# Vill-Lab/2023-TIFS-ISTVT

Hardware: AMD Instinct MI355X
Metric: clips/sec (BxTx3x224x224 fwd+bwd) (higher is better)
Workload: dtype bf16; 1 GPU; C2: B=32/GPU T=8 224x224 full ISTVT (Xception stem + 12-layer DSTTr) train step (fwd+bwd+grad all-reduce+SGD), random-init weights; global_batch=32, frames=8, size=224, depth=12, parallelism=dp1, early_allreduce=False, attn_fp8=False, dead_row_elimination=False, final_norm_class_rows_only=False, optimizer=SGD(momentum 0.9) fused, step_graphs=False

## Files before the change

2023-tifs-istvt_amd/build.py:

```python
import os
import subprocess
import sys
from concurrent.futures import ThreadPoolExecutor

HERE = os.path.dirname(os.path.abspath(__file__))
CSRC = os.path.join(HERE, 'csrc')
OBJ = os.path.join(CSRC, 'build')
LIB = os.path.join(HERE, 'libistvt_hip.so')
INCLUDE = os.path.join(os.path.dirname(HERE), 'include')
HIPCC = os.environ.get('HIPCC', '/opt/rocm/bin/hipcc')
FLAGS = ['--offload-arch=gfx950', '-O3', '-fPIC', '-std=c++17', '-Wno-unused-result', '-Wno-inline-asm', '-ffp-contract=fast', '-I', INCLUDE] + os.environ.get('ISTVT_EXTRA_HIPCC_FLAGS', '').split()


def _sources():
    return sorted(f for f in os.listdir(CSRC) if f.endswith('.hip'))


def _newest_header():
    headers = [os.path.join(CSRC, f) for f in os.listdir(CSRC) if f.endswith('.h')] + [os.path.join(INCLUDE, 'istvt_hip.h')]
    return max(os.path.getmtime(h) for h in headers)


def _compile(src):
    obj = os.path.join(OBJ, src[:-4] + '.o')
    path = os.path.join(CSRC, src)
    cmd = [HIPCC] + FLAGS + ['-Rpass-analysis=kernel-resource-usage', '-c', path, '-o', obj]
    r = subprocess.run(cmd, capture_output=True, text=True)
    if r.returncode != 0:
        raise RuntimeError('hipcc failed for %s:\n%s' % (src, r.stderr[-6000:]))
    _check_no_spills(src, r.stderr)
    return obj


NO_SPILL_KERNELS = ('gemm256q_kernel', 'gemm256t_kernel', 'gemm256t_group_kernel', 'pw_bwd_kernel')


def _check_no_spills(src, remarks):
    name = None
    for line in remarks.splitlines():
        if 'Function Name:' in line:
            name = line.split('Function Name:')[1].split()[0]
        elif 'ScratchSize [bytes/lane]:' in line and name and any(k in name for k in NO_SPILL_KERNELS):
            n = int(line.split('ScratchSize [bytes/lane]:')[1].split()[0])
            if n != 0:
                raise RuntimeError('%s: kernel %s spills %d bytes/lane to scratch; it must not (see build.py)' % (src, name, n))


def build(force: bool = False, verbose: bool = False) -> str:
    os.makedirs(OBJ, exist_ok=True)
    srcs = _sources()
    hdr = _newest_header()
    todo = []
    for s in srcs:
        obj = os.path.join(OBJ, s[:-4] + '.o')
        if force or not os.path.exists(obj) or os.path.getmtime(obj) < max(os.path.getmtime(os.path.join(CSRC, s)), hdr):
            todo.append(s)
    if verbose:
        print('compiling', todo)
    if todo:
        with ThreadPoolExecutor(max_workers=min(6, len(todo))) as ex:
            list(ex.map(_compile, todo))
    objs = [os.path.join(OBJ, s[:-4] + '.o') for s in srcs]
    if todo or not os.path.exists(LIB):
        cmd = [HIPCC, '--offload-arch=gfx950', '-shared', '-fPIC', '-o', LIB] + objs
        r = subprocess.run(cmd, capture_output=True, text=True)
        if r.returncode != 0:
            raise RuntimeError('link failed:\n' + r.stderr[-6000:])
    return LIB


if __name__ == '__main__':
    print(build(force='--force' in sys.argv, verbose=True))
```

2023-tifs-istvt_amd/csrc/conv_dense.hip:

```cpp
#include "common.h"
#include "u8_view.h"
#include <type_traits>

namespace {

__device__ __forceinline__ bf16x8 ld_frag(const bf16_t* p) { return *reinterpret_cast<const bf16x8*>(p); }
__device__ __forceinline__ bf16x8 zero_frag() {
    bf16x8 f;
#pragma unroll
    for (int i = 0; i < 8; ++i) f[i] = (bf16_t)0.0f;
    return f;
}
__device__ __forceinline__ f32x4 mma16(const bf16x8& a, const bf16x8& b, const f32x4& c) {
    return __builtin_amdgcn_mfma_f32_16x16x32_bf16(a, b, c, 0, 0, 0);
}

template <typename T>
__device__ __forceinline__ void conv1_mac_store(const float* v, const float* __restrict__ w, T* __restrict__ out) {
#pragma unroll
    for (int c8 = 0; c8 < 4; ++c8) {
        float o[8];
#pragma unroll
        for (int j = 0; j < 8; ++j) {
            const float* wc = w + (c8 * 8 + j) * 27;
            float a = 0.f;
#pragma unroll
            for (int k = 0; k < 27; ++k) a = fmaf(wc[k], v[k], a);
            o[j] = a;
        }
        store8(out + c8 * 8, o);
    }
}

template <typename T>
__global__ __launch_bounds__(256) void conv1_fwd_kernel(const float* __restrict__ x, const float* __restrict__ w,
                                                        T* __restrict__ u1, long Mo, int S, int Ho, int Wo) {
    const long m = (long)blockIdx.x * 256 + threadIdx.x;
    if (m >= Mo) return;
    const int xo = (int)(m % Wo), yo = (int)((m / Wo) % Ho);
    const long f = m / ((long)Wo * Ho);
    float v[27];
#pragma unroll
    for (int ci = 0; ci < 3; ++ci)
#pragma unroll
        for (int dy = 0; dy < 3; ++dy) {
            const float* row = x + ((f * 3 + ci) * S + 2 * yo + dy) * S + 2 * xo;
#pragma unroll
            for (int dx = 0; dx < 3; ++dx) v[ci * 9 + dy * 3 + dx] = row[dx];
        }
    conv1_mac_store(v, w, u1 + m * 32);
}

struct Conv1Mac {
    static __device__ __forceinline__ int slot(int dy, int dx, int ci) { return ci * 9 + dy * 3 + dx; }
    template <typename T>
    static __device__ __forceinline__ void emit(const float* v, const float* __restrict__ w, T* __restrict__ out) {
        int w0 = 0;
        asm volatile("" : "+s"(w0));
        conv1_mac_store(v, w + w0, out);
    }
};

struct Conv1Col {
    static __device__ __forceinline__ int slot(int dy, int dx, int ci) { return (dy * 3 + dx) * 3 + ci; }
    template <typename T>
    static __device__ __forceinline__ void emit(const float* v, const float*, T* __restrict__ out) {
#pragma unroll
        for (int c = 0; c < 4; ++c) {
            float t[8];
#pragma unroll
            for (int i = 0; i < 8; ++i) t[i] = c * 8 + i < 27 ? v[c * 8 + i] : 0.f;
            store8(out + c * 8, t);
        }
    }
};

template <typename Sink, typename T>
__global__ __launch_bounds__(256) void conv1_u8_kernel(const uint8_t* __restrict__ x, const int* __restrict__ view,
                                                       const float* __restrict__ mean, const float* __restrict__ stdv,
                                                       const float* __restrict__ w, T* __restrict__ out, long total,
                                                       int Hs, int Ws, int S, int Ho, int R, int ngroups) {
    extern __shared__ __align__(16) unsigned char smem[];
    float* lut = reinterpret_cast<float*>(smem);
    unsigned char* sb = smem + 3 * 256 * sizeof(float);
    const int tid = threadIdx.x;
    const int grp = (int)(blockIdx.x % ngroups);
    const long f = blockIdx.x / ngroups;
    const int yb = grp * R;
    const int rows = min(R, Ho - yb);
    const U8View vw = u8_view_of(view, f, Hs, Ws, S);
    u8_fill_lut(lut, mean, stdv, tid, 256);
    const int pitch = u8_row_pitch(S), rstride = Ws * 3;
    const long g0 = ((f * Hs + vw.y0 + 2 * yb) * (long)Ws + vw.x0) * 3;
    const int lead0 = u8_stage_rows(x, total, g0, rstride, 2 * rows + 1, S, sb, pitch, tid, 256);
    __syncthreads();
    const int nout = rows * Ho;
    for (int o = tid; o < nout; o += 256) {
        const int yl = o / Ho, xo = o - yl * Ho;
        float v[27];
#pragma unroll
        for (int dy = 0; dy < 3; ++dy) {
            const int rr = 2 * yl + dy;
            const unsigned char* row = sb + rr * pitch + u8_row_lead(lead0, rr, rstride);
#pragma unroll
            for (int dx = 0; dx < 3; ++dx) {
                const unsigned char* px = row + u8_view_px(2 * xo + dx, S, vw.flip);
#pragma unroll
                for (int ci = 0; ci < 3; ++ci) v[Sink::slot(dy, dx, ci)] = lut[ci * 256 + px[ci]];
            }
        }
        Sink::emit(v, w, out + ((f * Ho + yb) * (long)Ho + o) * 32);
    }
}

__global__ __launch_bounds__(256, 2) void conv2_fwd_kernel(const bf16_t* __restrict__ u1, const float* __restrict__ bnp,
                                                           const bf16_t* __restrict__ w, bf16_t* __restrict__ u2, long Mo,
                                                           int H, int W, int Ho, int Wo, int ngroups) {
    const int tid = threadIdx.x, lane = tid & 63, wave = tid >> 6;
    const int r = lane & 15, g = lane >> 4;
    __shared__ bf16x8 wl3[9 * 64];
    bf16x8 wf[9][3];
#pragma unroll
    for (int tap = 0; tap < 9; ++tap) {
#pragma unroll
        for (int nt = 0; nt < 3; ++nt)
            wf[tap][nt] = ld_frag(w + (16 * (r >> 2) + 4 * nt + (r & 3)) * 288 + tap * 32 + 8 * g);
        if (wave == 0) wl3[tap * 64 + lane] = ld_frag(w + (16 * (r >> 2) + 4 * 3 + (r & 3)) * 288 + tap * 32 + 8 * g);
    }
    __syncthreads();
    float mu[8], sc[8], be[8];
    load8(bnp + 8 * g, mu);
    load8(bnp + 2 * 32 + 8 * g, sc);
    load8(bnp + 3 * 32 + 8 * g, be);
    constexpr int RSEG = 9;
    const int nstrips = (Wo + 15) / 16, nsegs = (Ho + RSEG - 1) / RSEG;
    const long nitems = (long)(Mo / ((long)Ho * Wo)) * nstrips * nsegs;
    bf16x8 ring[3][3];
    for (long it = (long)blockIdx.x * 4 + wave; it < nitems; it += (long)gridDim.x * 4) {
        const int seg = (int)(it % nsegs);
        const int strip = (int)((it / nsegs) % nstrips);
        const long f = it / ((long)nsegs * nstrips);
        const int xo = strip * 16 + r;
        const bool ok = xo < Wo;
        const int xc = ok ? xo : Wo - 1;
        const int y0 = seg * RSEG;
        auto load_row = [&](int yi, bf16x8 (&dst)[3]) {
            const int yc = yi < H ? yi : H - 1;
            const bf16_t* sp = u1 + ((f * H + yc) * W + xc) * 32 + 8 * g;
#pragma unroll
            for (int dx = 0; dx < 3; ++dx) {
                const bf16x8 raw = ld_frag(sp + dx * 32);
#pragma unroll
                for (int j = 0; j < 8; ++j)
                    dst[dx][j] = (bf16_t)fmaxf(((float)raw[j] - mu[j]) * sc[j] + be[j], 0.f);
            }
        };
        load_row(y0, ring[0]);
        load_row(y0 + 1, ring[1]);
#pragma unroll
        for (int k = 0; k < RSEG; ++k) {
            const int yo = y0 + k;
            if (yo < Ho) {
                load_row(yo + 2, ring[(k + 2) % 3]);
                f32x4 acc[4];
#pragma unroll
                for (int nt = 0; nt < 4; ++nt) acc[nt] = f32x4{0.f, 0.f, 0.f, 0.f};
                int lo = lane;
                asm volatile("" : "+v"(lo));
#pragma unroll
                for (int dy = 0; dy < 3; ++dy)
#pragma unroll
                    for (int dx = 0; dx < 3; ++dx) {
                        const bf16x8& xf = ring[(k + dy) % 3][dx];
#pragma unroll
                        for (int nt = 0; nt < 3; ++nt) acc[nt] = mma16(wf[dy * 3 + dx][nt], xf, acc[nt]);
                        acc[3] = mma16(wl3[(dy * 3 + dx) * 64 + lo], xf, acc[3]);
                    }
                if (ok) {
                    bf16x8 o0, o1;
#pragma unroll
                    for (int i = 0; i < 4; ++i) {
                        o0[i] = (bf16_t)acc[0][i]; o0[4 + i] = (bf16_t)acc[1][i];
                        o1[i] = (bf16_t)acc[2][i]; o1[4 + i] = (bf16_t)acc[3][i];
                    }
                    bf16_t* dst = u2 + (((f * Ho + yo) * Wo) + xo) * 64 + 16 * g;
                    *reinterpret_cast<bf16x8*>(dst) = o0;
                    *reinterpret_cast<bf16x8*>(dst + 8) = o1;
                }
            }
        }
    }
}

__global__ __launch_bounds__(256, 2) void conv2_dgrad_kernel(const bf16_t* __restrict__ du2, const bf16_t* __restrict__ w,
                                                             const bf16_t* __restrict__ u1, const float* __restrict__ bnp,
                                                             bf16_t* __restrict__ dz1, long Mi, int H, int W, int Ho,
                                                             int Wo, int ngroups) {
    __shared__ bf16_t wt[9 * 32 * 64];
    const int tid = threadIdx.x, lane = tid & 63, wave = tid >> 6;
    const int r = lane & 15, g = lane >> 4;
    for (int i = tid; i < 64 * 36; i += 256) {
        const int co = i / 36, k8 = (i % 36) * 8;
        const bf16x8 v = ld_frag(w + co * 288 + k8);
#pragma unroll
        for (int j = 0; j < 8; ++j) wt[(k8 + j) * 64 + co] = v[j];
    }
    __syncthreads();
    bf16x8 wf[9][2][2];
#pragma unroll
    for (int tap = 3; tap < 9; ++tap)
#pragma unroll
        for (int ks = 0; ks < 2; ++ks)
#pragma unroll
            for (int nt = 0; nt < 2; ++nt)
                wf[tap][ks][nt] = ld_frag(wt + (tap * 32 + 8 * (r >> 2) + 4 * nt + (r & 3)) * 64 + 32 * ks + 8 * g);
    const int wrow = 8 * (r >> 2) + (r & 3), wcol = 8 * g;
    constexpr int RSEG = 9;
    const int nstrips = (W + 15) / 16, nsegs = (H + RSEG - 1) / RSEG;
    const long nitems = (long)(Mi / ((long)H * W)) * nstrips * nsegs;
    bf16x8 ring[3][3][2];
    for (long it = (long)blockIdx.x * 4 + wave; it < nitems; it += (long)gridDim.x * 4) {
        const int seg = (int)(it % nsegs);
        const int strip = (int)((it / nsegs) % nstrips);
        const long f = it / ((long)nsegs * nstrips);
        const int xi = strip * 16 + r;
        const int y0 = seg * RSEG;
        auto load_row = [&](int yo, bf16x8 (&dst)[3][2]) {
            const bool rowok = yo >= 0 && yo < Ho;
#pragma unroll
            for (int dx = 0; dx < 3; ++dx) {
                const int xo = xi - dx;
                const bool in = rowok && xo >= 0 && xo < Wo;
                const bf16_t* sp = du2 + ((f * Ho + yo) * Wo + xo) * 64 + 8 * g;
                dst[dx][0] = in ? ld_frag(sp) : zero_frag();
                dst[dx][1] = in ? ld_frag(sp + 32) : zero_frag();
            }
        };
        load_row(y0 - 2, ring[(RSEG * 3 - 2) % 3]);
        load_row(y0 - 1, ring[(RSEG * 3 - 1) % 3]);
#pragma unroll
        for (int k = 0; k < RSEG; ++k) {
            const int yi = y0 + k;
            if (yi < H) {
            load_row(yi, ring[k % 3]);
            const bool ok = xi < W;
            const long m = (f * H + yi) * W + (ok ? xi : W - 1);
            const bf16x8 uraw = ld_frag(u1 + m * 32 + 8 * g);
            f32x4 acc[2] = {f32x4{0.f, 0.f, 0.f, 0.f}, f32x4{0.f, 0.f, 0.f, 0.f}};
#pragma unroll
            for (int dyo = 2; dyo >= 1; --dyo) {
#pragma unroll
                for (int dx = 0; dx < 3; ++dx)
#pragma unroll
                    for (int ks = 0; ks < 2; ++ks)
#pragma unroll
                        for (int nt = 0; nt < 2; ++nt)
                            acc[nt] = mma16(wf[dyo * 3 + dx][ks][nt], ring[(k + 3 - dyo) % 3][dx][ks], acc[nt]);
            }
            int wo = wrow;
            asm volatile("" : "+v"(wo));
#pragma unroll
            for (int dx = 0; dx < 3; ++dx)
#pragma unroll
                for (int ks = 0; ks < 2; ++ks)
#pragma unroll
                    for (int nt = 0; nt < 2; ++nt)
                        acc[nt] = mma16(ld_frag(wt + (dx * 32 + wo + 4 * nt) * 64 + 32 * ks + wcol), ring[k % 3][dx][ks], acc[nt]);
            if (ok) {
                float mu[8], sc[8], be[8];
                load8(bnp + 8 * g, mu);
                load8(bnp + 2 * 32 + 8 * g, sc);
                load8(bnp + 3 * 32 + 8 * g, be);
                bf16x8 o;
#pragma unroll
                for (int j = 0; j < 8; ++j) {
                    const float z = ((float)uraw[j] - mu[j]) * sc[j] + be[j];
                    o[j] = (bf16_t)(z > 0.f ? acc[j >> 2][j & 3] : 0.f);
                }
                *reinterpret_cast<bf16x8*>(dz1 + m * 32 + 8 * g) = o;
            }
            }
        }
    }
}

constexpr int WG_PX = 32;
constexpr int DIMG_PITCH = 64 * 2 + 16;
constexpr int AIMG_PITCH = 32 * 2 + 16;
constexpr int AIMG_ROWS = WG_PX + 2;

__device__ __forceinline__ bf16x8 tr_frag(const char* img, int pitch, int k0, int col16, int r) {
    typedef short4v __attribute__((address_space(3))) * lds_ptr;
    typedef short short8v __attribute__((ext_vector_type(8)));
    const int q = r >> 2, pp = r & 3;
    const char* pa = img + (k0 + q) * pitch + (col16 + 4 * pp) * 2;
    const char* pb = pa + 4 * pitch;
    const short4v lo = __builtin_amdgcn_ds_read_tr16_b64_v4i16((lds_ptr)(pa));
    const short4v hi = __builtin_amdgcn_ds_read_tr16_b64_v4i16((lds_ptr)(pb));
    short8v s;
    s[0] = lo[0]; s[1] = lo[1]; s[2] = lo[2]; s[3] = lo[3]; s[4] = hi[0]; s[5] = hi[1]; s[6] = hi[2]; s[7] = hi[3];
    return __builtin_bit_cast(bf16x8, s);
}

__global__ __launch_bounds__(256) void conv2_wgrad_kernel(const bf16_t* __restrict__ du2, const bf16_t* __restrict__ u1,
                                                          const float* __restrict__ bnp, float* __restrict__ slabs,
                                                          int Fr, int H, int W, int Ho, int Wo, int nchunks) {
    __shared__ __attribute__((aligned(16))) char dimg[WG_PX * DIMG_PITCH];
    __shared__ __attribute__((aligned(16))) char aimg[3 * AIMG_ROWS * AIMG_PITCH];
    const int tid = threadIdx.x, lane = tid & 63, wave = tid >> 6;
    const int r = lane & 15, g = lane >> 4;
    const int cpr = (Wo + WG_PX - 1) / WG_PX;
    f32x4 acc[9][2];
#pragma unroll
    for (int t = 0; t < 9; ++t) acc[t][0] = acc[t][1] = f32x4{0.f, 0.f, 0.f, 0.f};
    const int dpx = tid >> 3, dpc = tid & 7;
    float mu[8], sc[8], be[8];
    load8(bnp + 8 * (tid & 3), mu);
    load8(bnp + 2 * 32 + 8 * (tid & 3), sc);
    load8(bnp + 3 * 32 + 8 * (tid & 3), be);
    bf16x8 dreg, areg[2];
    auto gload = [&](int ch) {
        const int x0 = (ch % cpr) * WG_PX;
        const int rowi = ch / cpr;
        const int yo = rowi % Ho;
        const long f = rowi / Ho;
        dreg = zero_frag();
        if (x0 + dpx < Wo) dreg = ld_frag(du2 + ((f * Ho + yo) * Wo + x0 + dpx) * 64 + dpc * 8);
#pragma unroll
        for (int k = 0; k < 2; ++k) {
            const int i = tid + 256 * k;
            const int px = (i >> 2) % AIMG_ROWS, dy = (i >> 2) / AIMG_ROWS;
            areg[k] = zero_frag();
            if (i < 3 * AIMG_ROWS * 4 && x0 + px < W)
                areg[k] = ld_frag(u1 + ((f * H + yo + dy) * W + x0 + px) * 32 + (tid & 3) * 8);
        }
    };
    int ch = blockIdx.x;
    if (ch < nchunks) gload(ch);
    for (; ch < nchunks; ch += gridDim.x) {
        const int x0 = (ch % cpr) * WG_PX;
        *reinterpret_cast<bf16x8*>(dimg + dpx * DIMG_PITCH + dpc * 16) = dreg;
#pragma unroll
        for (int k = 0; k < 2; ++k) {
            const int i = tid + 256 * k;
            const int px = (i >> 2) % AIMG_ROWS, dy = (i >> 2) / AIMG_ROWS;
            if (i < 3 * AIMG_ROWS * 4) {
                bf16x8 v = zero_frag();
                if (x0 + px < W) {
#pragma unroll
                    for (int j = 0; j < 8; ++j) v[j] = (bf16_t)fmaxf(((float)areg[k][j] - mu[j]) * sc[j] + be[j], 0.f);
                }
                *reinterpret_cast<bf16x8*>(aimg + (dy * AIMG_ROWS + px) * AIMG_PITCH + (tid & 3) * 16) = v;
            }
        }
        __syncthreads();
        if (ch + (int)gridDim.x < nchunks) gload(ch + gridDim.x);
        const bf16x8 df = tr_frag(dimg, DIMG_PITCH, 8 * g, 16 * wave, r);
#pragma unroll
        for (int tap = 0; tap < 9; ++tap) {
            const char* ab = aimg + ((tap / 3) * AIMG_ROWS + (tap % 3)) * AIMG_PITCH;
#pragma unroll
            for (int ct = 0; ct < 2; ++ct) acc[tap][ct] = mma16(df, tr_frag(ab, AIMG_PITCH, 8 * g, 16 * ct, r), acc[tap][ct]);
        }
        __syncthreads();
    }
    float* out = slabs + (long)blockIdx.x * 64 * 288;
#pragma unroll
    for (int tap = 0; tap < 9; ++tap)
#pragma unroll
        for (int ct = 0; ct < 2; ++ct)
#pragma unroll
            for (int i = 0; i < 4; ++i) out[(16 * wave + 4 * g + i) * 288 + tap * 32 + 16 * ct + r] = acc[tap][ct][i];
}

constexpr int C1_PX = 128;
constexpr int C1_PITCH = 32 * 2 + 16;

struct C1Row {
    long f;
    int yo;
};

template <typename TD>
__device__ __forceinline__ C1Row c1_load_du1(const TD* __restrict__ du1, int row, int Ho, int Wo, int tid, bf16x8 (&dreg)[2]) {
    const C1Row c{row / Ho, row % Ho};
#pragma unroll
    for (int k = 0; k < 2; ++k) {
        const int i = tid + 256 * k;
        const int px = i >> 2, pc = i & 3;
        dreg[k] = zero_frag();
        if (px < Wo) {
            float v[8];
            load8(du1 + ((c.f * Ho + c.yo) * Wo + px) * 32 + pc * 8, v);
#pragma unroll
            for (int j = 0; j < 8; ++j) dreg[k][j] = (bf16_t)v[j];
        }
    }
    return c;
}

__device__ __forceinline__ void c1_store_du1(char* dimg, int tid, const bf16x8 (&dreg)[2]) {
#pragma unroll
    for (int k = 0; k < 2; ++k) {
        const int i = tid + 256 * k;
        *reinterpret_cast<bf16x8*>(dimg + (i >> 2) * C1_PITCH + (i & 3) * 16) = dreg[k];
    }
}

__device__ __forceinline__ void c1_store_patch(char* pimg, int px, int k0, const float (&v)[16]) {
    bf16x8 p0, p1;
#pragma unroll
    for (int j = 0; j < 8; ++j) { p0[j] = (bf16_t)v[j]; p1[j] = (bf16_t)v[8 + j]; }
    *reinterpret_cast<bf16x8*>(pimg + px * C1_PITCH + k0 * 2) = p0;
    *reinterpret_cast<bf16x8*>(pimg + px * C1_PITCH + k0 * 2 + 16) = p1;
}

__device__ __forceinline__ f32x4 c1_mma(const char* dimg, const char* pimg, int tid, f32x4 acc) {
    const int lane = tid & 63, wave = tid >> 6, r = lane & 15, g = lane >> 4;
#pragma unroll
    for (int ks = 0; ks < C1_PX / 32; ++ks)
        acc = mma16(tr_frag(dimg, C1_PITCH, 32 * ks + 8 * g, 16 * (wave >> 1), r),
                    tr_frag(pimg, C1_PITCH, 32 * ks + 8 * g, 16 * (wave & 1), r), acc);
    return acc;
}

__device__ __forceinline__ void c1_store_slab(float* __restrict__ slabs, int tid, const f32x4& acc) {
    const int lane = tid & 63, wave = tid >> 6, r = lane & 15, g = lane >> 4;
    float* out = slabs + (long)blockIdx.x * 32 * 32;
#pragma unroll
    for (int i = 0; i < 4; ++i) out[(16 * (wave >> 1) + 4 * g + i) * 32 + 16 * (wave & 1) + r] = acc[i];
}

template <typename TD>
__global__ __launch_bounds__(256) void conv1_wgrad_kernel(const TD* __restrict__ du1, const float* __restrict__ x,
                                                          float* __restrict__ slabs, int S, int Ho, int Wo, int nrows) {
    __shared__ __attribute__((aligned(16))) char dimg[C1_PX * C1_PITCH];
    __shared__ __attribute__((aligned(16))) char pimg[C1_PX * C1_PITCH];
    const int tid = threadIdx.x;
    const int ppx = tid >> 1, pk0 = (tid & 1) * 16;
    f32x4 acc = f32x4{0.f, 0.f, 0.f, 0.f};
    bf16x8 dreg[2];
    float xreg[16];
    auto gload = [&](int row) {
        const C1Row c = c1_load_du1(du1, row, Ho, Wo, tid, dreg);
#pragma unroll
        for (int j = 0; j < 16; ++j) {
            const int k = pk0 + j;
            const int ci = k / 9, dy = (k % 9) / 3, dx = k % 3;
            xreg[j] = 0.f;
            if (k < 27 && ppx < Wo) xreg[j] = x[((c.f * 3 + ci) * S + 2 * c.yo + dy) * S + 2 * ppx + dx];
        }
    };
    int row = blockIdx.x;
    if (row < nrows) gload(row);
    for (; row < nrows; row += gridDim.x) {
        c1_store_du1(dimg, tid, dreg);
        c1_store_patch(pimg, ppx, pk0, xreg);
        __syncthreads();
        if (row + (int)gridDim.x < nrows) gload(row + gridDim.x);
        acc = c1_mma(dimg, pimg, tid, acc);
        __syncthreads();
    }
    c1_store_slab(slabs, tid, acc);
}

constexpr int C1B_MAXS = 2 * C1_PX + 2;
constexpr int C1B_CPR = (C1B_MAXS * 3 + 30) >> 4;
constexpr int C1B_PITCH = C1B_CPR * 16;
static_assert(3 * C1B_CPR <= 256, "one 16-byte piece per thread");

template <typename TD>
__global__ __launch_bounds__(256) void conv1_wgrad_u8_kernel(const TD* __restrict__ du1, const uint8_t* __restrict__ x,
                                                             const int* __restrict__ view, const float* __restrict__ mean,
                                                             const float* __restrict__ stdv, float* __restrict__ slabs,
                                                             long total, int Hs, int Ws, int S, int Ho, int Wo, int nrows) {
    __shared__ __attribute__((aligned(16))) char dimg[C1_PX * C1_PITCH];
    __shared__ __attribute__((aligned(16))) char pimg[C1_PX * C1_PITCH];
    __shared__ __attribute__((aligned(16))) unsigned char sb[3 * C1B_PITCH];
    __shared__ float lut[3 * 256];
    const int tid = threadIdx.x;
    const int ppx = tid & (C1_PX - 1), pk0 = (tid >> 7) * 16;
    const int brow = tid / C1B_CPR, bc = tid - brow * C1B_CPR;
    const int rstride = Ws * 3, len = S * 3;
    u8_fill_lut(lut, mean, stdv, tid, 256);
    f32x4 acc = f32x4{0.f, 0.f, 0.f, 0.f};
    bf16x8 dreg[2];
    uint4 breg = make_uint4(0u, 0u, 0u, 0u);
    int lead0 = 0, flip = 0, lead0n = 0, flipn = 0;
    auto gload = [&](int row) {
        const C1Row c = c1_load_du1(du1, row, Ho, Wo, tid, dreg);
        const U8View vw = u8_view_of(view, c.f, Hs, Ws, S);
        const long g0 = ((c.f * Hs + vw.y0 + 2 * c.yo) * (long)Ws + vw.x0) * 3;
        lead0n = (int)((reinterpret_cast<uintptr_t>(x) + (uintptr_t)g0) & 15);
        flipn = vw.flip;
        if (brow < 3) {
            const int lead = u8_row_lead(lead0n, brow, rstride);
            if (16 * bc < lead + len) breg = u8_load16(x, g0 + (long)brow * rstride - lead + 16L * bc, total);
        }
    };
    auto patch = [&](auto k0) {
        constexpr int K0 = decltype(k0)::value;
        int rowoff[3], pxoff[3];
#pragma unroll
        for (int d = 0; d < 3; ++d) {
            rowoff[d] = d * C1B_PITCH + u8_row_lead(lead0, d, rstride);
            pxoff[d] = u8_view_px(2 * ppx + d, S, flip);
        }
        float v[16];
#pragma unroll
        for (int j = 0; j < 16; ++j) {
            const int k = K0 + j;
            const int ci = k / 9, dy = (k % 9) / 3, dx = k % 3;
            v[j] = 0.f;
            if (k < 27 && ppx < Wo) v[j] = lut[ci * 256 + sb[rowoff[dy] + pxoff[dx] + ci]];
        }
        c1_store_patch(pimg, ppx, K0, v);
    };
    int row = blockIdx.x;
    if (row < nrows) gload(row);
    for (; row < nrows; row += gridDim.x) {
        c1_store_du1(dimg, tid, dreg);
        if (brow < 3) *reinterpret_cast<uint4*>(sb + brow * C1B_PITCH + 16 * bc) = breg;
        lead0 = lead0n, flip = flipn;
        __syncthreads();
        if (pk0 == 0) patch(std::integral_constant<int, 0>()); else patch(std::integral_constant<int, 16>());
        if (row + (int)gridDim.x < nrows) gload(row + gridDim.x);
        __syncthreads();
        acc = c1_mma(dimg, pimg, tid, acc);
        __syncthreads();
    }
    c1_store_slab(slabs, tid, acc);
}

inline int wave_grid(int ngroups, int per_cu) {
    const int need = (ngroups + 3) / 4;
    const int cap = 256 * per_cu;
    return need < cap ? (need > 0 ? need : 1) : cap;
}

}

extern "C" int istvt_conv1_fwd(const float* x, const float* w, void* u1, int Fr, int S, int dtype, hipStream_t stream) {
    if (Fr <= 0 || S < 3) return ISTVT_ERR_SHAPE;
    const int Ho = (S - 3) / 2 + 1;
    const long Mo = (long)Fr * Ho * Ho;
    DISPATCH_DTYPE(dtype, hipLaunchKernelGGL((conv1_fwd_kernel<T>), dim3((unsigned)((Mo + 255) / 256)), dim3(256), 0,
                                             stream, x, w, (T*)u1, Mo, S, Ho, Ho));
    return istvt_check_launch();
}

static inline bool u8_view_args_ok(const void* x, long total, int Hs, int Ws, const float* mean, const float* stdv, int Fr,
                                   int S) {
    if (Fr <= 0 || S < 3 || !x || !mean || !stdv) return false;
    if (Hs < S || Ws < S || Hs > 16384 || Ws > 16384) return false;
    return total >= (long)Fr * Hs * Ws * 3;
}

template <typename Sink>
static int conv1_u8_launch(const void* x, long total, int Hs, int Ws, const int* view, const float* mean, const float* stdv,
                           const float* w, void* out, int Fr, int S, int dtype, hipStream_t stream) {
    if (!u8_view_args_ok(x, total, Hs, Ws, mean, stdv, Fr, S) || S > 4096 || !out) return ISTVT_ERR_SHAPE;
    const int Ho = (S - 3) / 2 + 1;
    const int pitch = u8_row_pitch(S);
    int R = 1;
    double best = 0.0;
    for (int r = 1; r <= 16 && r <= Ho; ++r) {
        if ((2L * r + 1) * pitch > 48 * 1024) break;
        const double eff = r < 4 ? 0.0 : (double)(r * Ho) / (double)(((r * Ho + 255) / 256) * 256);
        if (r < 4 || eff > best + 1e-9) best = eff, R = r;
    }
    const int ngroups = (Ho + R - 1) / R;
    const long nblocks = (long)Fr * ngroups;
    if (nblocks > 0x7fffffffL) return ISTVT_ERR_SHAPE;
    const size_t lds = 3 * 256 * sizeof(float) + (size_t)(2 * R + 1) * pitch;
    DISPATCH_DTYPE(dtype, hipLaunchKernelGGL((conv1_u8_kernel<Sink, T>), dim3((unsigned)nblocks), dim3(256), lds, stream,
                                             (const uint8_t*)x, view, mean, stdv, w, (T*)out, total, Hs, Ws, S, Ho, R, ngroups));
    return istvt_check_launch();
}

extern "C" int istvt_conv1_fwd_u8_view(const void* x, long total, int Hs, int Ws, const int* view, const float* mean,
                                       const float* stdv, const float* w, void* u1, int Fr, int S, int dtype,
                                       hipStream_t stream) {
    if (!w) return ISTVT_ERR_SHAPE;
    return conv1_u8_launch<Conv1Mac>(x, total, Hs, Ws, view, mean, stdv, w, u1, Fr, S, dtype, stream);
}

extern "C" int istvt_conv1_fwd_u8(const void* x, const float* mean, const float* stdv, const float* w, void* u1, int Fr,
                                  int S, int dtype, hipStream_t stream) {
    return istvt_conv1_fwd_u8_view(x, (long)Fr * S * S * 3, S, S, nullptr, mean, stdv, w, u1, Fr, S, dtype, stream);
}

extern "C" int istvt_im2col_conv1_u8(const void* x, long total, int Hs, int Ws, const int* view, const float* mean,
                                     const float* stdv, void* col, int Fr, int S, int dtype, hipStream_t stream) {
    return conv1_u8_launch<Conv1Col>(x, total, Hs, Ws, view, mean, stdv, nullptr, col, Fr, S, dtype, stream);
}

extern "C" int istvt_conv2_fwd(const void* u1, const float* bnp, const void* w, void* u2, int Fr, int H, int W,
                               hipStream_t stream) {
    if (Fr <= 0 || H < 3 || W < 3 || !bnp) return ISTVT_ERR_SHAPE;
    const int Ho = H - 2, Wo = W - 2;
    const long Mo = (long)Fr * Ho * Wo;
    if (Mo / 16 + 1 > 0x7fffffffL) return ISTVT_ERR_SHAPE;
    const int ngroups = (int)((Mo + 15) / 16);
    const long items = (long)Fr * ((Wo + 15) / 16) * ((Ho + 8) / 9);
    hipLaunchKernelGGL(conv2_fwd_kernel, dim3(wave_grid((int)(items < 0x7fffffffL ? items : 0x7fffffffL), 2)), dim3(256), 0, stream, (const bf16_t*)u1, bnp,
                       (const bf16_t*)w, (bf16_t*)u2, Mo, H, W, Ho, Wo, ngroups);
    return istvt_check_launch();
}

extern "C" int istvt_conv2_dgrad(const void* du2, const void* w, const void* u1, const float* bnp, void* dz1, int Fr,
                                 int H, int W, hipStream_t stream) {
    if (Fr <= 0 || H < 3 || W < 3 || !bnp) return ISTVT_ERR_SHAPE;
    const long Mi = (long)Fr * H * W;
    if (Mi / 16 + 1 > 0x7fffffffL) return ISTVT_ERR_SHAPE;
    const int ngroups = (int)((Mi + 15) / 16);
    const long items = (long)Fr * ((W + 15) / 16) * ((H + 8) / 9);
    hipLaunchKernelGGL(conv2_dgrad_kernel, dim3(wave_grid((int)(items < 0x7fffffffL ? items : 0x7fffffffL), 2)), dim3(256), 0, stream, (const bf16_t*)du2,
                       (const bf16_t*)w, (const bf16_t*)u1, bnp, (bf16_t*)dz1, Mi, H, W, H - 2, W - 2, ngroups);
    return istvt_check_launch();
}

extern "C" int istvt_conv2_wgrad_slabs() { return 768; }

extern "C" int istvt_conv2_wgrad(const void* du2, const void* u1, const float* bnp, float* slabs, float* dw, int Fr,
                                 int H, int W, hipStream_t stream) {
    if (Fr <= 0 || H < 3 || W < 3 || !bnp || !slabs) return ISTVT_ERR_SHAPE;
    const int Ho = H - 2, Wo = W - 2;
    const long nch = (long)Fr * Ho * ((Wo + WG_PX - 1) / WG_PX);
    if (nch > 0x7fffffffL) return ISTVT_ERR_SHAPE;
    const int cap = istvt_conv2_wgrad_slabs();
    const int grid = nch < cap ? (int)nch : cap;
    hipLaunchKernelGGL(conv2_wgrad_kernel, dim3(grid), dim3(256), 0, stream, (const bf16_t*)du2, (const bf16_t*)u1, bnp,
                       slabs, Fr, H, W, Ho, Wo, (int)nch);
    int rc = istvt_check_launch();
    if (rc != ISTVT_OK) return rc;
    const int n = 64 * 288;
    return istvt_rows_reduce_add(slabs, grid, 1, n, dw, nullptr, nullptr, stream);
}

extern "C" int istvt_conv1_wgrad_slabs() { return 1024; }

template <typename Launch>
static int conv1_wgrad_launch(float* slabs, float* dw, int Fr, int S, hipStream_t stream, Launch launch) {
    if (Fr <= 0 || S < 3 || !slabs) return ISTVT_ERR_SHAPE;
    const int Ho = (S - 3) / 2 + 1;
    if (Ho > C1_PX) return ISTVT_ERR_SHAPE;
    const long nrows = (long)Fr * Ho;
    if (nrows > 0x7fffffffL) return ISTVT_ERR_SHAPE;
    const int cap = istvt_conv1_wgrad_slabs();
    const int grid = nrows < cap ? (int)nrows : cap;
    int rc = launch(grid, Ho, (int)nrows);
    if (rc == ISTVT_OK) rc = istvt_check_launch();
    if (rc != ISTVT_OK) return rc;
    return istvt_rows_reduce_add(slabs, grid, 1, 1024, dw, nullptr, nullptr, stream);
}

extern "C" int istvt_conv1_wgrad(const void* du1, const float* x, float* slabs, float* dw, int Fr, int S, int dtype,
                                 hipStream_t stream) {
    return conv1_wgrad_launch(slabs, dw, Fr, S, stream, [&](int grid, int Ho, int nrows) {
        DISPATCH_DTYPE(dtype, hipLaunchKernelGGL((conv1_wgrad_kernel<T>), dim3(grid), dim3(256), 0, stream, (const T*)du1, x,
                                                 slabs, S, Ho, Ho, nrows));
        return ISTVT_OK;
    });
}

extern "C" int istvt_conv1_wgrad_u8(const void* du1, const void* x, long total, int Hs, int Ws, const int* view,
                                    const float* mean, const float* stdv, float* slabs, float* dw, int Fr, int S, int dtype,
                                    hipStream_t stream) {
    if (!u8_view_args_ok(x, total, Hs, Ws, mean, stdv, Fr, S) || !du1 || !dw) return ISTVT_ERR_SHAPE;
    return conv1_wgrad_launch(slabs, dw, Fr, S, stream, [&](int grid, int Ho, int nrows) {
        DISPATCH_DTYPE(dtype, hipLaunchKernelGGL((conv1_wgrad_u8_kernel<T>), dim3(grid), dim3(256), 0, stream, (const T*)du1,
                                                 (const uint8_t*)x, view, mean, stdv, slabs, total, Hs, Ws, S, Ho, Ho, nrows));
        return ISTVT_OK;
    });
}
```

Before: 633.3 clips/s.

## Add LDS ring-buffered async row prefetch for conv2 forward and dgrad

```diff
diff --git a/2023-tifs-istvt_amd/build.py b/2023-tifs-istvt_amd/build.py
--- a/2023-tifs-istvt_amd/build.py
+++ b/2023-tifs-istvt_amd/build.py
@@ -32,7 +32,8 @@
     return obj
 
 
-NO_SPILL_KERNELS = ('gemm256q_kernel', 'gemm256t_kernel', 'gemm256t_group_kernel', 'pw_bwd_kernel')
+NO_SPILL_KERNELS = ('gemm256q_kernel', 'gemm256t_kernel', 'gemm256t_group_kernel', 'pw_bwd_kernel',
+                    'conv2_fwd_ring_kernel', 'conv2_dgrad_ring_kernel')
 
 
 def _check_no_spills(src, remarks):
diff --git a/2023-tifs-istvt_amd/csrc/conv_dense.hip b/2023-tifs-istvt_amd/csrc/conv_dense.hip
--- a/2023-tifs-istvt_amd/csrc/conv_dense.hip
+++ b/2023-tifs-istvt_amd/csrc/conv_dense.hip
@@ -1,5 +1,6 @@
 #include "common.h"
 #include "u8_view.h"
+#include <cstdlib>
 #include <type_traits>
 
 namespace {
@@ -192,6 +193,212 @@
     }
 }
 
+constexpr unsigned C2R_OOB = 0x80000000u;
+
+__device__ __forceinline__ __amdgpu_buffer_rsrc_t c2r_frame_rsrc(const bf16_t* base, long f, int frame_bytes) {
+    const unsigned long long u = (unsigned long long)base + (unsigned long long)f * (unsigned)frame_bytes;
+    const unsigned lo = __builtin_amdgcn_readfirstlane((unsigned)u), hi = __builtin_amdgcn_readfirstlane((unsigned)(u >> 32));
+    return __builtin_amdgcn_make_buffer_rsrc((void*)(((unsigned long long)hi << 32) | lo), 0, frame_bytes, 0x00020000u);
+}
+
+template <int N> __device__ __forceinline__ void c2r_wait_vm() { asm volatile("s_waitcnt vmcnt(%0)" ::"n"(N) : "memory"); }
+
+template <int DEPTH, int NPC, int NST>
+__device__ __forceinline__ void c2r_wait_row(int nst) {
+    static_assert(DEPTH <= 6 && (DEPTH - 1) * NPC + DEPTH * NST <= 63, "the ladder below; vmcnt is a 6-bit field");
+    constexpr int B = (DEPTH - 1) * NPC;
+    if (nst >= DEPTH) c2r_wait_vm<B + DEPTH * NST>();
+    else if (nst == 5) c2r_wait_vm<B + 5 * NST>();
+    else if (nst == 4) c2r_wait_vm<B + 4 * NST>();
+    else if (nst == 3) c2r_wait_vm<B + 3 * NST>();
+    else if (nst == 2) c2r_wait_vm<B + 2 * NST>();
+    else if (nst == 1) c2r_wait_vm<B + 1 * NST>();
+    else c2r_wait_vm<B>();
+}
+
+struct C2RWalk {
+    int nstrips, nsegs, dseg, dstrip, df;
+    __device__ __forceinline__ void init(long stride, int nstrips_, int nsegs_) {
+        nstrips = nstrips_, nsegs = nsegs_;
+        dseg = (int)(stride % nsegs), dstrip = (int)((stride / nsegs) % nstrips), df = (int)(stride / ((long)nsegs * nstrips));
+    }
+};
+struct C2RItem {
+    int seg, strip, f;
+    __device__ __forceinline__ void init(long it, const C2RWalk& wk) {
+        seg = (int)(it % wk.nsegs), strip = (int)((it / wk.nsegs) % wk.nstrips), f = (int)(it / ((long)wk.nsegs * wk.nstrips));
+    }
+    __device__ __forceinline__ void step(const C2RWalk& wk) {
+        seg += wk.dseg;
+        if (seg >= wk.nsegs) seg -= wk.nsegs, ++strip;
+        strip += wk.dstrip;
+        if (strip >= wk.nstrips) strip -= wk.nstrips, ++f;
+        f += wk.df;
+    }
+};
+
+template <int CH, int RSEG, int NEXTRA, int YLEAD, int XLEAD>
+struct C2RCursor {
+    static constexpr int ROW_BYTES = 18 * CH * 2;
+    static constexpr int NPC = (ROW_BYTES + 1023) / 1024;
+    static constexpr bool TAIL4 = ROW_BYTES - (NPC - 1) * 1024 <= 256;
+    static constexpr int LDS_BYTES = (NPC - 1) * 1024 + (TAIL4 ? 256 : 1024);
+    const bf16_t* src;
+    int Fr, Hs, Ws, Hitem, lane;
+    C2RItem item;
+    int row, nrows, y;
+    unsigned off;
+    unsigned voff[NPC];
+    bool live;
+    __amdgpu_buffer_rsrc_t rs;
+
+    __device__ __forceinline__ void set() {
+        live = item.f < Fr;
+        const int x0 = item.strip * 16 + XLEAD;
+        y = item.seg * RSEG + YLEAD;
+        nrows = min(RSEG, Hitem - item.seg * RSEG) + NEXTRA;
+        row = 0;
+        off = (unsigned)((y * Ws + x0) * (CH * 2));
+        rs = c2r_frame_rsrc(src, live ? item.f : 0, Hs * Ws * CH * 2);
+#pragma unroll
+        for (int p = 0; p < NPC; ++p) {
+            const int b = p * 1024 + lane * (p == NPC - 1 && TAIL4 ? 4 : 16);
+            const int px = x0 + b / (CH * 2);
+            voff[p] = live && b < ROW_BYTES && px >= 0 && px < Ws ? (unsigned)b : C2R_OOB;
+        }
+    }
+    __device__ __forceinline__ void issue(unsigned dst) const {
+        const bool rowok = y >= 0 && y < Hs;
+#pragma unroll
+        for (int p = 0; p < NPC; ++p) {
+            const unsigned v = rowok ? voff[p] + off : C2R_OOB;
+            if (p == NPC - 1 && TAIL4) dma4_lds(rs, dst + p * 1024, v, 0);
+            else dma16_lds(rs, dst + p * 1024, v, 0);
+        }
+    }
+    __device__ __forceinline__ void next(const C2RWalk& wk) {
+        off += (unsigned)(Ws * CH * 2);
+        ++y;
+        if (++row == nrows) {
+            if (live) item.step(wk);
+            set();
+        }
+    }
+};
+
+constexpr int C2F_DEPTH = 6;
+constexpr int C2F_SLOT = 1280;
+
+__global__ __launch_bounds__(256, 2) void conv2_fwd_ring_kernel(const bf16_t* __restrict__ u1, const float* __restrict__ bnp,
+                                                                const bf16_t* __restrict__ w, bf16_t* __restrict__ u2,
+                                                                long Mo, int H, int W, int Ho, int Wo) {
+    constexpr int RSEG = 9, DEPTH = C2F_DEPTH, NPC = 2, NST = 2;
+    typedef C2RCursor<32, RSEG, 2, 0, 0> Cursor;
+    static_assert(Cursor::NPC == NPC && Cursor::LDS_BYTES == C2F_SLOT, "two pieces per row");
+    __shared__ __attribute__((aligned(16))) char smem[9 * 64 * 16 + 4 * DEPTH * C2F_SLOT];
+    bf16x8* wl3 = reinterpret_cast<bf16x8*>(smem);
+    const int tid = threadIdx.x, lane = tid & 63;
+    const int wave = __builtin_amdgcn_readfirstlane(tid >> 6);
+    const int r = lane & 15, g = lane >> 4;
+    bf16x8 wf[9][3];
+#pragma unroll
+    for (int tap = 0; tap < 9; ++tap) {
+#pragma unroll
+        for (int nt = 0; nt < 3; ++nt)
+            wf[tap][nt] = ld_frag(w + (16 * (r >> 2) + 4 * nt + (r & 3)) * 288 + tap * 32 + 8 * g);
+        if (wave == 0) wl3[tap * 64 + lane] = ld_frag(w + (16 * (r >> 2) + 4 * 3 + (r & 3)) * 288 + tap * 32 + 8 * g);
+    }
+    __syncthreads();
+    float mu[8], sc[8], be[8];
+    load8(bnp + 8 * g, mu);
+    load8(bnp + 2 * 32 + 8 * g, sc);
+    load8(bnp + 3 * 32 + 8 * g, be);
+    const int nstrips = (Wo + 15) / 16, nsegs = (Ho + RSEG - 1) / RSEG;
+    const long nitems = (long)(Mo / ((long)Ho * Wo)) * nstrips * nsegs;
+    const long first = (long)blockIdx.x * 4 + wave, stride = (long)gridDim.x * 4;
+    typedef __attribute__((address_space(3))) void lds_v;
+    const char* ringp = smem + 9 * 64 * 16 + wave * (DEPTH * C2F_SLOT);
+    const unsigned ring0 = (unsigned)(__SIZE_TYPE__)(lds_v*)smem + 9 * 64 * 16 + wave * (DEPTH * C2F_SLOT);
+    const int Fr = (int)(Mo / ((long)Ho * Wo));
+    C2RWalk wk;
+    wk.init(stride, nstrips, nsegs);
+    C2RItem rd;
+    rd.init(first, wk);
+    Cursor cur;
+    cur.src = u1, cur.Fr = Fr, cur.Hs = H, cur.Ws = W, cur.Hitem = Ho, cur.lane = lane, cur.item = rd;
+    cur.set();
+    int wslot = 0;
+    auto issue = [&]() {
+        cur.issue(ring0 + wslot * C2F_SLOT);
+        cur.next(wk);
+        wslot = wslot + 1 == DEPTH ? 0 : wslot + 1;
+    };
+    if (first < nitems) {
+#pragma unroll
+        for (int i = 0; i < DEPTH; ++i) issue();
+    }
+    int hist = 0, rslot = 0;
+    bf16x8 ring[3][3];
+    auto take_row = [&](bf16x8 (&dst)[3]) {
+        c2r_wait_row<DEPTH, NPC, NST>(__builtin_popcount(hist));
+        const char* sp = ringp + rslot * C2F_SLOT + r * 64 + g * 16;
+        bf16x8 raw[3];
+#pragma unroll
+        for (int dx = 0; dx < 3; ++dx) raw[dx] = *reinterpret_cast<const bf16x8*>(sp + dx * 64);
+        asm volatile("s_waitcnt lgkmcnt(0)" ::: "memory");
+        issue();
+        rslot = rslot + 1 == DEPTH ? 0 : rslot + 1;
+        hist = (hist << 1) & ((1 << DEPTH) - 1);
+#pragma unroll
+        for (int dx = 0; dx < 3; ++dx)
+#pragma unroll
+            for (int j = 0; j < 8; ++j) dst[dx][j] = (bf16_t)fmaxf(((float)raw[dx][j] - mu[j]) * sc[j] + be[j], 0.f);
+    };
+    for (; rd.f < Fr; rd.step(wk)) {
+        const long f = rd.f;
+        const int xo = rd.strip * 16 + r;
+        const bool ok = xo < Wo;
+        const int y0 = rd.seg * RSEG;
+        const int nout = min(RSEG, Ho - y0);
+        take_row(ring[0]);
+        take_row(ring[1]);
+#pragma unroll
+        for (int k = 0; k < RSEG; ++k) {
+            const int yo = y0 + k;
+            if (k < nout) {
+                take_row(ring[(k + 2) % 3]);
+                f32x4 acc[4];
+#pragma unroll
+                for (int nt = 0; nt < 4; ++nt) acc[nt] = f32x4{0.f, 0.f, 0.f, 0.f};
+                int lo = lane;
+                asm volatile("" : "+v"(lo));
+#pragma unroll
+                for (int dy = 0; dy < 3; ++dy)
+#pragma unroll
+                    for (int dx = 0; dx < 3; ++dx) {
+                        const bf16x8& xf = ring[(k + dy) % 3][dx];
+#pragma unroll
+                        for (int nt = 0; nt < 3; ++nt) acc[nt] = mma16(wf[dy * 3 + dx][nt], xf, acc[nt]);
+                        acc[3] = mma16(wl3[(dy * 3 + dx) * 64 + lo], xf, acc[3]);
+                    }
+                if (ok) {
+                    bf16x8 o0, o1;
+#pragma unroll
+                    for (int i = 0; i < 4; ++i) {
+                        o0[i] = (bf16_t)acc[0][i]; o0[4 + i] = (bf16_t)acc[1][i];
+                        o1[i] = (bf16_t)acc[2][i]; o1[4 + i] = (bf16_t)acc[3][i];
+                    }
+                    bf16_t* dst = u2 + (((f * Ho + yo) * Wo) + xo) * 64 + 16 * g;
+                    *reinterpret_cast<bf16x8*>(dst) = o0;
+                    *reinterpret_cast<bf16x8*>(dst + 8) = o1;
+                }
+                hist |= 1;
+            }
+        }
+    }
+    asm volatile("s_waitcnt vmcnt(0)" ::: "memory");
+}
+
 __global__ __launch_bounds__(256, 2) void conv2_dgrad_kernel(const bf16_t* __restrict__ du2, const bf16_t* __restrict__ w,
                                                              const bf16_t* __restrict__ u1, const float* __restrict__ bnp,
                                                              bf16_t* __restrict__ dz1, long Mi, int H, int W, int Ho,
@@ -282,6 +489,144 @@
             }
         }
     }
+}
+
+constexpr int C2D_DEPTH = 5;
+constexpr int C2D_SLOT = 2304 + 1024;
+constexpr int C2D_WT_KEEP = 3 * 32 * 64 * 2;
+constexpr int C2D_BN = C2D_WT_KEEP + 4 * C2D_DEPTH * C2D_SLOT;
+constexpr int C2D_LDS = C2D_BN + 3 * 32 * 4;
+static_assert(C2D_LDS >= 9 * 32 * 64 * 2 && 2 * C2D_LDS <= 160 * 1024, "the whole image fits at first; two workgroups per CU");
+
+__global__ __launch_bounds__(256, 2) void conv2_dgrad_ring_kernel(const bf16_t* __restrict__ du2, const bf16_t* __restrict__ w,
+                                                                  const bf16_t* __restrict__ u1, const float* __restrict__ bnp,
+                                                                  bf16_t* __restrict__ dz1, long Mi, int H, int W, int Ho,
+                                                                  int Wo) {
+    constexpr int RSEG = 9, DEPTH = C2D_DEPTH, NPC = 4, NST = 1;
+    typedef C2RCursor<64, RSEG, 2, -2, -2> Cursor;
+    static_assert(Cursor::NPC + 1 == NPC && Cursor::LDS_BYTES + 1024 == C2D_SLOT, "three pieces of du2 and one of u1 per row");
+    __shared__ __attribute__((aligned(16))) char smem[C2D_LDS];
+    bf16_t* wt = reinterpret_cast<bf16_t*>(smem);
+    float* bnl = reinterpret_cast<float*>(smem + C2D_BN);
+    const int tid = threadIdx.x, lane = tid & 63;
+    const int wave = __builtin_amdgcn_readfirstlane(tid >> 6);
+    const int r = lane & 15, g = lane >> 4;
+    for (int i = tid; i < 64 * 36; i += 256) {
+        const int co = i / 36, k8 = (i % 36) * 8;
+        const bf16x8 v = ld_frag(w + co * 288 + k8);
+#pragma unroll
+        for (int j = 0; j < 8; ++j) wt[(k8 + j) * 64 + co] = v[j];
+    }
+    if (tid < 96) bnl[tid] = bnp[(tid < 32 ? 0 : 32) + tid];
+    __syncthreads();
+    bf16x8 wf[9][2][2];
+#pragma unroll
+    for (int tap = 3; tap < 9; ++tap)
+#pragma unroll
+        for (int ks = 0; ks < 2; ++ks)
+#pragma unroll
+            for (int nt = 0; nt < 2; ++nt)
+                wf[tap][ks][nt] = ld_frag(wt + (tap * 32 + 8 * (r >> 2) + 4 * nt + (r & 3)) * 64 + 32 * ks + 8 * g);
+    __syncthreads();
+    const int wrow = 8 * (r >> 2) + (r & 3), wcol = 8 * g;
+    const int nstrips = (W + 15) / 16, nsegs = (H + RSEG - 1) / RSEG;
+    const int Fr = (int)(Mi / ((long)H * W));
+    const long first = (long)blockIdx.x * 4 + wave, stride = (long)gridDim.x * 4;
+    typedef __attribute__((address_space(3))) void lds_v;
+    const char* ringp = smem + C2D_WT_KEEP + wave * (DEPTH * C2D_SLOT);
+    const unsigned ring0 = (unsigned)(__SIZE_TYPE__)(lds_v*)smem + C2D_WT_KEEP + wave * (DEPTH * C2D_SLOT);
+    C2RWalk wk;
+    wk.init(stride, nstrips, nsegs);
+    C2RItem rd;
+    rd.init(first, wk);
+    Cursor cur;
+    cur.src = du2, cur.Fr = Fr, cur.Hs = Ho, cur.Ws = Wo, cur.Hitem = H, cur.lane = lane, cur.item = rd;
+    cur.set();
+    int wslot = 0;
+    auto issue = [&]() {
+        const unsigned dst = ring0 + wslot * C2D_SLOT;
+        cur.issue(dst);
+        const __amdgpu_buffer_rsrc_t ru = c2r_frame_rsrc(u1, cur.live ? cur.item.f : 0, H * W * 64);
+        const int x0 = cur.item.strip * 16;
+        const bool uok = cur.live && cur.row >= 2 && x0 + (lane >> 2) < W;
+        dma16_lds(ru, dst + Cursor::LDS_BYTES, uok ? (unsigned)((cur.y * W + x0) * 64 + lane * 16) : C2R_OOB, 0);
+        cur.next(wk);
+        wslot = wslot + 1 == DEPTH ? 0 : wslot + 1;
+    };
+    if (rd.f < Fr) {
+#pragma unroll
+        for (int i = 0; i < DEPTH; ++i) issue();
+    }
+    int hist = 0, rslot = 0;
+    bf16x8 ring[3][3][2];
+    auto take_row = [&](bf16x8 (&dst)[3][2], bf16x8& uraw) {
+        c2r_wait_row<DEPTH, NPC, NST>(__builtin_popcount(hist));
+        const char* sp = ringp + rslot * C2D_SLOT;
+#pragma unroll
+        for (int dx = 0; dx < 3; ++dx)
+#pragma unroll
+            for (int ks = 0; ks < 2; ++ks) dst[dx][ks] = *reinterpret_cast<const bf16x8*>(sp + (r - dx + 2) * 128 + ks * 64 + g * 16);
+        uraw = *reinterpret_cast<const bf16x8*>(sp + Cursor::LDS_BYTES + r * 64 + g * 16);
+        asm volatile("s_waitcnt lgkmcnt(0)" ::: "memory");
+        issue();
+        rslot = rslot + 1 == DEPTH ? 0 : rslot + 1;
+        hist = (hist << 1) & ((1 << DEPTH) - 1);
+    };
+    for (; rd.f < Fr; rd.step(wk)) {
+        const long f = rd.f;
+        const int xi = rd.strip * 16 + r;
+        const int y0 = rd.seg * RSEG;
+        const int nin = min(RSEG, H - y0);
+        bf16x8 uraw;
+        take_row(ring[(RSEG * 3 - 2) % 3], uraw);
+        take_row(ring[(RSEG * 3 - 1) % 3], uraw);
+#pragma unroll
+        for (int k = 0; k < RSEG; ++k) {
+            const int yi = y0 + k;
+            if (k < nin) {
+            take_row(ring[k % 3], uraw);
+            const bool ok = xi < W;
+            const long m = (f * H + yi) * W + (ok ? xi : W - 1);
+            f32x4 acc[2] = {f32x4{0.f, 0.f, 0.f, 0.f}, f32x4{0.f, 0.f, 0.f, 0.f}};
+#pragma unroll
+            for (int dyo = 2; dyo >= 1; --dyo) {
+#pragma unroll
+                for (int dx = 0; dx < 3; ++dx)
+#pragma unroll
+                    for (int ks = 0; ks < 2; ++ks)
+#pragma unroll
+                        for (int nt = 0; nt < 2; ++nt)
+                            acc[nt] = mma16(wf[dyo * 3 + dx][ks][nt], ring[(k + 3 - dyo) % 3][dx][ks], acc[nt]);
+            }
+            int wo = wrow;
+            asm volatile("" : "+v"(wo));
+#pragma unroll
+            for (int dx = 0; dx < 3; ++dx)
+#pragma unroll
+                for (int ks = 0; ks < 2; ++ks)
+#pragma unroll
+                    for (int nt = 0; nt < 2; ++nt)
+                        acc[nt] = mma16(ld_frag(wt + (dx * 32 + wo + 4 * nt) * 64 + 32 * ks + wcol), ring[k % 3][dx][ks], acc[nt]);
+            if (ok) {
+                float mu[8], sc[8], be[8];
+                int bo = 8 * g;
+                asm volatile("" : "+v"(bo));
+                load8(bnl + bo, mu);
+                load8(bnl + 32 + bo, sc);
+                load8(bnl + 64 + bo, be);
+                bf16x8 o;
+#pragma unroll
+                for (int j = 0; j < 8; ++j) {
+                    const float z = ((float)uraw[j] - mu[j]) * sc[j] + be[j];
+                    o[j] = (bf16_t)(z > 0.f ? acc[j >> 2][j & 3] : 0.f);
+                }
+                *reinterpret_cast<bf16x8*>(dz1 + m * 32 + 8 * g) = o;
+            }
+            hist |= 1;
+            }
+        }
+    }
+    asm volatile("s_waitcnt vmcnt(0)" ::: "memory");
 }
 
 constexpr int WG_PX = 32;
@@ -532,6 +877,12 @@
     c1_store_slab(slabs, tid, acc);
 }
 
+constexpr long C2R_MAX_FRAME = 1L << 30;
+inline bool conv_dense_ring() {
+    const char* v = getenv("ISTVT_CONV_DENSE_RING");
+    return !(v && v[0] == '0' && v[1] == '\0');
+}
+
 inline int wave_grid(int ngroups, int per_cu) {
     const int need = (ngroups + 3) / 4;
     const int cap = 256 * per_cu;
@@ -603,7 +954,12 @@
     if (Mo / 16 + 1 > 0x7fffffffL) return ISTVT_ERR_SHAPE;
     const int ngroups = (int)((Mo + 15) / 16);
     const long items = (long)Fr * ((Wo + 15) / 16) * ((Ho + 8) / 9);
-    hipLaunchKernelGGL(conv2_fwd_kernel, dim3(wave_grid((int)(items < 0x7fffffffL ? items : 0x7fffffffL), 2)), dim3(256), 0, stream, (const bf16_t*)u1, bnp,
+    if (conv_dense_ring() && (long)H * W * 64 <= C2R_MAX_FRAME) {
+        hipLaunchKernelGGL(conv2_fwd_ring_kernel, dim3(wave_grid((int)(items < 0x7fffffffL ? items : 0x7fffffffL), 2)), dim3(256), 0, stream,
+                           (const bf16_t*)u1, bnp, (const bf16_t*)w, (bf16_t*)u2, Mo, H, W, Ho, Wo);
+        return istvt_check_launch();
+    }
+    hipLaunchKernelGGL(conv2_fwd_kernel,dim3(wave_grid((int)(items < 0x7fffffffL ? items : 0x7fffffffL), 2)), dim3(256), 0, stream, (const bf16_t*)u1, bnp,
                        (const bf16_t*)w, (bf16_t*)u2, Mo, H, W, Ho, Wo, ngroups);
     return istvt_check_launch();
 }
@@ -615,6 +971,11 @@
     if (Mi / 16 + 1 > 0x7fffffffL) return ISTVT_ERR_SHAPE;
     const int ngroups = (int)((Mi + 15) / 16);
     const long items = (long)Fr * ((W + 15) / 16) * ((H + 8) / 9);
+    if (conv_dense_ring() && (long)H * W * 128 <= C2R_MAX_FRAME) {
+        hipLaunchKernelGGL(conv2_dgrad_ring_kernel, dim3(wave_grid((int)(items < 0x7fffffffL ? items : 0x7fffffffL), 2)), dim3(256), 0, stream,
+                           (const bf16_t*)du2, (const bf16_t*)w, (const bf16_t*)u1, bnp, (bf16_t*)dz1, Mi, H, W, H - 2, W - 2);
+        return istvt_check_launch();
+    }
     hipLaunchKernelGGL(conv2_dgrad_kernel, dim3(wave_grid((int)(items < 0x7fffffffL ? items : 0x7fffffffL), 2)), dim3(256), 0, stream, (const bf16_t*)du2,
                        (const bf16_t*)w, (const bf16_t*)u1, bnp, (bf16_t*)dz1, Mi, H, W, H - 2, W - 2, ngroups);
     return istvt_check_launch();
```

Measured after the change: 635.3 clips/s (median of 6 runs). Within noise of the previous version (+0.3%).
